# zifeo/distributed-sgd

Measured on NVIDIA H100. Metric: sgd_samples_per_sec, higher is better.
Workload: dtype f64

## Files before the change

distributed_sgd_b200/csrc/dsgd_api.cu:

```cuda
#include "../../include/dsgd.h"

#include <cuda.h>
#include <cuda_runtime.h>
#include <dlfcn.h>
#include <nccl.h>

#include <algorithm>
#include <cmath>
#include <cstdarg>
#include <cstdio>
#include <cstring>
#include <limits>
#include <mutex>
#include <string>
#include <type_traits>
#include <utility>
#include <vector>

#include "dsgd_kernels.cuh"
#include "dsgd_persistent.cuh"
#include "dsgd_stream.cuh"
#include "dsgd_async.cuh"
#include "dsgd_metrics.cuh"
#include "dsgd_calibrate.cuh"
// ... 2599 lines not shown
  if (!nccl().ok) return fail(nullptr, DSGD_ERR_NCCL, "%s", nccl().why.c_str());
  ncclUniqueId u;
  ncclResult_t r = nccl().GetUniqueId(&u);
  if (r != ncclSuccess) return fail(nullptr, DSGD_ERR_NCCL, "ncclGetUniqueId: %s", nccl().GetErrorString(r));
  memcpy(id, &u, sizeof u);
  return DSGD_OK;
}

extern "C" int dsgd_comm_init(dsgd_ctx *ctx, const uint8_t id[DSGD_UNIQUE_ID_BYTES]) {
  if (!ctx) return DSGD_ERR_INVALID;
  NEED(id, DSGD_ERR_INVALID, "dsgd_comm_init: id is NULL");
  NEED(!ctx->comm, DSGD_ERR_STATE, "dsgd_comm_init: communicator already initialised");
  CU(cudaSetDevice(ctx->device));
  ncclUniqueId u;
  memcpy(&u, id, sizeof u);
  NEED(nccl().ok, DSGD_ERR_NCCL, "%s", nccl().why.c_str());
  NC(nccl().CommInitRank(&ctx->comm, ctx->world, u, ctx->rank));
  return DSGD_OK;
}

constexpr int kPCons = 8, kPUpd = 6, kPStages = 8, kPStagePairs = 2560, kPMaxChunks = 128;
using PSmem = PersistSmem<kPCons, kPUpd, kPStages, kPStagePairs, kPMaxChunks>;
constexpr int kPersistForms = 28, kPersistFused = 24;
constexpr bool pf_multi(int f) { return f >= kPersistFused; }
constexpr int pf_weight(int f) { return pf_multi(f) ? kUnweighted : f / 8; }
constexpr bool pf_l1(int f) { return (f & 4) != 0; }
template <int... F>
static void *const *persist_forms(std::integer_sequence<int, F...>) {
  static void *const k[] = {(void *)k_sync_persistent<kPCons, kPUpd, kPStages, kPStagePairs, kPMaxChunks, pf_multi(F),
                                                      (F & 2) != 0, (F & 1) != 0, pf_l1(F), pf_weight(F)>...};
  return k;
}
static void *const *const kPersistKernels = persist_forms(std::make_integer_sequence<int, kPersistForms>{});
static int persist_form(bool multi, bool avg, bool lr_table, bool l1, int weight) {
  if (multi) return kPersistFused + 2 * avg + lr_table;
  return 8 * weight + 4 * l1 + 2 * avg + lr_table;
}
static size_t persist_smem(int f) {
  return sizeof(PSmem) + (pf_weight(f) == kSampleWeighted ? sizeof(PersistSwSmem<kPStages>) : 0);
}
static bool persist_timeline() { static const bool v = getenv("DSGD_PERSIST_TIMELINE") != nullptr; return v; }

static int persist_prepare(dsgd_ctx *ctx, int64_t n_steps) {
  if (!ctx->p_ready) {
    const int64_t nv = (int64_t)ctx->dim + 2;
    const size_t vd = sizeof(double) * (size_t)nv;
    for (int i = 0; i < 2; ++i) CU(ctx->p_wbuf[i].alloc(nv));
    for (int i = 0; i < 3; ++i) {
      CU(ctx->p_gbuf[i].alloc(nv));
      CU(cudaMemsetAsync(ctx->p_gbuf[i], 0, vd, ctx->stream));
      CU(ctx->p_rec[i].alloc(nv));
      CU(cudaMemsetAsync(ctx->p_rec[i], 0, 2 * vd, ctx->stream));
    }
    CU(ctx->p_acc.alloc(3 * kAccStride));
    CU(ctx->p_bar.alloc(4));
    for (int f = 0; f < kPersistForms; ++f)
      CU(cudaFuncSetAttribute(kPersistKernels[f], cudaFuncAttributeMaxDynamicSharedMemorySize, (int)persist_smem(f)));
    ctx->p_ready = true;
  }
  int rc = ctx->p_hinge.grow(ctx, (int64_t)ctx->sm_count * n_steps, 4096 * (int64_t)ctx->sm_count);
  if (rc) return rc;
  if (weighting(ctx) == kSampleWeighted &&
      (rc = ctx->p_hcode.grow(ctx, (int64_t)ctx->sm_count * n_steps, 4096 * (int64_t)ctx->sm_count)))
    return rc;
  return ctx->p_loss_nrm.grow(ctx, 2 * n_steps, 2 * 4096);
}

static int persist_grid(const dsgd_ctx *ctx, int64_t batch) {
  const int g = ctx->grid_limit > 0 ? std::min(ctx->grid_limit, ctx->sm_count) : ctx->sm_count;
  if (cdiv(batch, kMaxRowsPerCta) > g) return 0;
  if (ctx->n_pairs >= (1ll << 31)) return 0;
  return g;
}
static bool persist_multi_fits(const dsgd_ctx *ctx, int G) {
  const int slice = (cdiv(ctx->dim + 1, G) + 31) & ~31;
  return slice <= (kPCons + kPUpd) * 32;
}

static cudaError_t persist_launch(dsgd_ctx *ctx, int form, int G, void **args) {
  void *fn = kPersistKernels[form];
  const size_t smem = persist_smem(form);
  if (ctx->grid_limit > 0) return cudaLaunchKernel(fn, dim3(G), dim3((kPCons + kPUpd + 1) * 32), args, smem, ctx->stream);
  return cudaLaunchCooperativeKernel(fn, dim3(G), dim3((kPCons + kPUpd + 1) * 32), args, smem, ctx->stream);
}

static size_t xblk_stride(const dsgd_ctx *ctx) { return (size_t)(ctx->dim + kReplicaPad); }
static size_t xblk_words(const dsgd_ctx *ctx) { return ((size_t)ctx->dim + 1 + 31) / 32; }
static size_t xblk_bm_offset(const dsgd_ctx *ctx) { return 2 * (size_t)kMaxWorld * 2 * xblk_stride(ctx); }
static size_t xblk_doubles(const dsgd_ctx *ctx) { return xblk_bm_offset(ctx) + (size_t)kMaxWorld * 2 * xblk_words(ctx); }

static int xblk_ensure(dsgd_ctx *ctx) {
  if (ctx->xblk) return DSGD_OK;
  CU(cudaSetDevice(ctx->device));
  CU(ctx->xblk.alloc((int64_t)xblk_doubles(ctx)));
  CU(cudaMemset(ctx->xblk, 0, sizeof(double) * xblk_doubles(ctx)));
  CU(ctx->x_stats.alloc(4));
  CU(cudaMemset(ctx->x_stats, 0, sizeof(unsigned long long) * 4));
  return DSGD_OK;
}

static int xllw_ensure(dsgd_ctx *ctx) {
  if (ctx->x_llw) return DSGD_OK;
  CU(ctx->x_llw.alloc(2 * 2 * (int64_t)xblk_stride(ctx)));
  CU(cudaMemsetAsync(ctx->x_llw, 0, 2 * 2 * sizeof(unsigned long long) * xblk_stride(ctx), ctx->stream));
  return DSGD_OK;
}

static bool xchg_complete(const dsgd_ctx *ctx) {
  if (ctx->world <= 1 || ctx->world > kMaxWorld || !ctx->xblk) return false;
  for (int r = 0; r < ctx->world; ++r)
    if (r != ctx->rank && !ctx->peer_x[r]) return false;
  return true;
}

static int persist_run(dsgd_ctx *ctx, bool multi, const int32_t *samples_dev, int64_t n_per_step, int64_t n_steps,
                       double lr, const double *lrs_host, double *losses_dev) {
  int rc = persist_prepare(ctx, n_steps);
  if (rc) return rc;
  const int G = persist_grid(ctx, n_per_step);
  NEED((uint64_t)G * (uint64_t)(n_steps + 2) < (1ull << 32), DSGD_ERR_INVALID, "dsgd_sync_steps: too many steps for one launch");
  PersistParams pp;
  memset(&pp, 0, sizeof pp);
  pp.rp16 = ctx->rp16; pp.pairs = ctx->pairs; pp.label = ctx->label; pp.samples = samples_dev;
  pp.n_steps = n_steps; pp.batch = (int32_t)n_per_step; pp.dim = ctx->dim;
  pp.wbuf[0] = ctx->p_wbuf[0]; pp.wbuf[1] = ctx->p_wbuf[1];
  for (int i = 0; i < 3; ++i) { pp.gbuf[i] = ctx->p_gbuf[i]; pp.rec[i] = ctx->p_rec[i]; }
  pp.d = ctx->d; pp.acc = ctx->p_acc; pp.bar = ctx->p_bar; pp.hinge = ctx->p_hinge; pp.losses = losses_dev;
  pp.loss_nrm = ctx->p_loss_nrm;
  pp.w_out = ctx->w; pp.w32_out = ctx->w32; pp.scal = ctx->scal;
  pp.abort_flag = reinterpret_cast<int *>(ctx->p_bar + 1);
  CU(cudaMemsetAsync(ctx->p_acc, 0, sizeof(unsigned long long) * 3 * kAccStride, ctx->stream));
  pp.lambda = ctx->lambda; pp.lr = lr; pp.world = 1;
  CU(cudaMemsetAsync(ctx->p_bar, 0, sizeof(unsigned) * 4, ctx->stream));
  if (persist_timeline()) {
    if (!ctx->p_tl) CU(ctx->p_tl.alloc(kTlWords));
    CU(cudaMemsetAsync(ctx->p_tl, 0, sizeof(long long) * kTlWords, ctx->stream));
    pp.tl = ctx->p_tl;
  }
  if (!multi) {
    k_rec_init<<<cdiv(ctx->dim, 256), 256, 0, ctx->stream>>>(ctx->w, ctx->dim, ctx->p_rec[0], ctx->p_rec[1], ctx->p_rec[2]);
    LAUNCHED();
    pp.k_den = 1.0;
    pp.timeout_cycles = 4000000000ll;
  } else {
    CU(cudaMemcpyAsync(ctx->p_wbuf[0], ctx->w, sizeof(double) * (size_t)ctx->dim, cudaMemcpyDeviceToDevice, ctx->stream));
    pp.k_den = (double)ctx->world;
    pp.timeout_cycles = 20000000000ll;
    pp.world = ctx->world; pp.rank = ctx->rank; pp.step_base = ctx->x_step;
    pp.xstride = (int)xblk_stride(ctx);
    pp.xwords = (int)xblk_words(ctx);
    for (int r = 0; r < ctx->world; ++r) {
      unsigned long long *blk = reinterpret_cast<unsigned long long *>((r == ctx->rank) ? ctx->xblk.p : ctx->peer_x[r].p);
      pp.xval[r] = blk;
      pp.xbm[r] = blk + xblk_bm_offset(ctx);
    }
    if ((rc = xllw_ensure(ctx))) return rc;
    pp.llw[0] = ctx->x_llw;
    pp.llw[1] = ctx->x_llw + 2 * xblk_stride(ctx);
    pp.xstats = ctx->x_stats;
  }
  if (ctx->avg_on) pp.avg = ctx->avg;
  if (lrs_host) {
    if ((rc = ctx->lrs.grow(ctx, n_steps, 1024))) return rc;
    CU(cudaMemcpyAsync(ctx->lrs, lrs_host, sizeof(double) * (size_t)n_steps, cudaMemcpyHostToDevice, ctx->stream));
    pp.lrs = ctx->lrs;
    pp.lr = 0.0;
  }
  void *args[] = {&pp};
  const bool l1 = !multi && ctx->lambda1 > 0.0;
  pp.lambda1 = l1 ? ctx->lambda1 : 0.0;
  pp.w_pos = ctx->cw_pos; pp.w_neg = ctx->cw_neg;
  const int weight = multi ? kUnweighted : weighting(ctx);
  if (weight == kSampleWeighted) { pp.sw = ctx->sw; pp.hcode = ctx->p_hcode; }
  const int form = persist_form(multi, ctx->avg_on, lrs_host != nullptr, l1, weight);
  cudaError_t launch_err = cudaSuccess;
  profiled(ctx, [&] { launch_err = persist_launch(ctx, form, G, args); });
  CU(launch_err);
  LAUNCHED();
  if (ctx->avg_on) ctx->avg_n += n_steps;
  if (multi) {
    ctx->x_step += n_steps + 6;
    ctx->x_steps_run += n_steps;
  }
  return DSGD_OK;
// ... 694 lines not shown
```

distributed_sgd_b200/csrc/dsgd_fixed.cuh:

```cuda
#pragma once
#include <cuda_runtime.h>
#include <stdint.h>

namespace dsgd {

constexpr int kAccStride = 16;
constexpr int kAccLimbs = 5;
constexpr int kAccWords = 2 * kAccLimbs + 1;
static_assert(kAccWords + 1 <= kAccStride, "acc_read loads the accumulator and one pad word");
__device__ __forceinline__ void red_add_u64(unsigned long long *p, unsigned long long v) {
  asm volatile("red.relaxed.gpu.global.add.u64 [%0], %1;" ::"l"(p), "l"(v) : "memory");
}
template <class Put>
__device__ __forceinline__ void acc_cut(double a, Put &&put) {
  double F[kAccLimbs - 1];
#pragma unroll
  for (int i = 0; i < kAccLimbs - 1; ++i) F[i] = floor(a * __longlong_as_double((1023ll + 40 * i) << 52));
  put(kAccLimbs - 1, F[0]);
#pragma unroll
  for (int i = 1; i < kAccLimbs - 1; ++i) put(kAccLimbs - 1 - i, F[i] - F[i - 1] * 0x1p40);
  put(0, rint(a * 0x1p160) - F[kAccLimbs - 2] * 0x1p40);
}
__device__ __forceinline__ void acc_push_one(unsigned long long *limbs, unsigned long long *ovf, double v) {
  if (!(fabs(v) < 4503599627370496.0)) {
    red_add_u64(ovf, 1ull);
    return;
  }
  const bool neg = v < 0.0;
  acc_cut(fabs(v), [&](int k, double limb) {
    if (limb != 0.0) {
      const unsigned long long u = (unsigned long long)(long long)limb;
      red_add_u64(limbs + k, neg ? (0ull - u) : u);
    }
  });
}
__device__ __forceinline__ void acc_push(unsigned long long *acc, double sd, double sn) {
  acc_push_one(acc, acc + 2 * kAccLimbs, sd);
  acc_push_one(acc + kAccLimbs, acc + 2 * kAccLimbs, sn);
}
__device__ __forceinline__ double acc_limb(unsigned long long q, int k) {
  return (double)(long long)q * __longlong_as_double((long long)(1023 - 160 + 40 * (k % kAccLimbs)) << 52);
}
__device__ __forceinline__ void acc_load(const unsigned long long *acc, int lane, unsigned long long &q0, unsigned long long &q1) {
  q0 = 0; q1 = 0;
  if (lane < (kAccWords + 1) / 2)
    asm volatile("ld.relaxed.gpu.global.v2.u64 {%0, %1}, [%2];" : "=l"(q0), "=l"(q1) : "l"(acc + 2 * lane) : "memory");
}
__device__ __forceinline__ void acc_sum(unsigned long long q0, unsigned long long q1, int lane, double &sd, double &sn) {
  const double lo = acc_limb(q0, 2 * lane), hi = acc_limb(q1, 2 * lane + 1), pair = lo + hi;
  const double s01 = __shfl_sync(0xffffffffu, pair, 0), s23 = __shfl_sync(0xffffffffu, pair, 1);
  const double s4 = __shfl_sync(0xffffffffu, lo, 2), n0 = __shfl_sync(0xffffffffu, hi, 2);
  const double n12 = __shfl_sync(0xffffffffu, pair, 3), n34 = __shfl_sync(0xffffffffu, pair, 4);
  sd = (s01 + s23) + s4;
  sn = (n0 + n12) + n34;
  if (__any_sync(0xffffffffu, lane == kAccWords / 2 && q0 != 0)) {
    sd = __longlong_as_double(0x7ff8000000000000ll);
    sn = sd;
  }
}
__device__ __forceinline__ void acc_read(const unsigned long long *acc, int lane, double &sd, double &sn) {
  unsigned long long q0, q1;
  acc_load(acc, lane, q0, q1);
  acc_sum(q0, q1, lane, sd, sn);
}
__device__ __forceinline__ void acc_load_l1(const unsigned long long *acc, int lane, unsigned long long &q, unsigned long long &o) {
  q = 0; o = 0;
  if (lane < kAccLimbs) asm volatile("ld.relaxed.gpu.global.u64 %0, [%1];" : "=l"(q) : "l"(acc + kAccWords + lane) : "memory");
  if (lane == 0) asm volatile("ld.relaxed.gpu.global.u64 %0, [%1];" : "=l"(o) : "l"(acc + 2 * kAccLimbs) : "memory");
}
__device__ __forceinline__ double acc_sum_l1(unsigned long long q, unsigned long long o, int lane) {
  const double v = acc_limb(q, lane);
  const double v0 = __shfl_sync(0xffffffffu, v, 0), v1 = __shfl_sync(0xffffffffu, v, 1), v2 = __shfl_sync(0xffffffffu, v, 2);
  const double v3 = __shfl_sync(0xffffffffu, v, 3), v4 = __shfl_sync(0xffffffffu, v, 4);
  const double a = (((v4 + v3) + v2) + v1) + v0;
  return __shfl_sync(0xffffffffu, o, 0) != 0ull ? __longlong_as_double(0x7ff8000000000000ll) : a;
}
__device__ __forceinline__ double acc_read_l1(const unsigned long long *acc, int lane) {
  unsigned long long q, o;
  acc_load_l1(acc, lane, q, o);
  return acc_sum_l1(q, o, lane);
}

constexpr int kLossLimbs = kAccLimbs + 1;
constexpr int kLossAccWords = kLossLimbs + 1;
constexpr unsigned long long kLimbMask = (1ull << 40) - 1;
__device__ __forceinline__ void acc_carry(unsigned long long (&q)[kLossLimbs]) {
#pragma unroll
  for (int i = 0; i < kLossLimbs - 1; ++i) {
    q[i + 1] += q[i] >> 40;
    q[i] &= kLimbMask;
  }
}
__device__ __forceinline__ void acc_add_local(unsigned long long (&lim)[kLossLimbs], unsigned long long &ovf, double v) {
  if (!(v >= 0.0 && v < 4503599627370496.0)) { ++ovf; return; }
  acc_cut(v, [&](int k, double limb) { lim[k] += (unsigned long long)(long long)limb; });
  acc_carry(lim);
}
__device__ __forceinline__ void acc_flush_local(unsigned long long *acc, const unsigned long long (&lim)[kLossLimbs],
                                                unsigned long long ovf) {
#pragma unroll
  for (int i = 0; i < kLossLimbs; ++i)
    if (lim[i]) red_add_u64(acc + i, lim[i]);
  if (ovf) red_add_u64(acc + kLossLimbs, ovf);
}
__device__ __forceinline__ double acc_value(const unsigned long long *acc) {
  if (acc[kLossLimbs] != 0ull) return __longlong_as_double(0x7ff8000000000000ll);
  unsigned long long q[kLossLimbs];
#pragma unroll
  for (int i = 0; i < kLossLimbs; ++i) q[i] = acc[i];
  acc_carry(q);
  double s = (double)q[kLossLimbs - 1] * 0x1p40;
#pragma unroll
  for (int i = kLossLimbs - 2; i >= 0; --i) s += (double)q[i] * __longlong_as_double((long long)(1023 - 160 + 40 * i) << 52);
  return s;
}

}
```

distributed_sgd_b200/csrc/dsgd_persistent.cuh:

```cuda
#pragma once
#include <cuda_runtime.h>
#include <stdint.h>

#include <type_traits>

#include "dsgd_fixed.cuh"
#include "dsgd_kernels.cuh"

namespace dsgd {

constexpr int kMaxWorld = 8;

struct PersistParams {
  const uint32_t *rp16;
  const uint2 *pairs;
  const int8_t *label;
  const int32_t *samples;
  int64_t n_steps;
  int32_t batch;
  int32_t dim;
  double *wbuf[2];
  double *gbuf[3];
  double2 *rec[3];
  const double *d;
// ... 77 lines not shown
__device__ __forceinline__ void st_relaxed_gpu(unsigned *p, unsigned v) {
  asm volatile("st.relaxed.gpu.global.u32 [%0], %1;" ::"l"(p), "r"(v) : "memory");
}
__device__ __forceinline__ void fence_acq_rel_gpu() { asm volatile("fence.acq_rel.gpu;" ::: "memory"); }
__device__ __forceinline__ void named_bar_sync(int id, int n_threads) {
  asm volatile("bar.sync %0, %1;" ::"r"(id), "r"(n_threads) : "memory");
}
__device__ __forceinline__ void named_bar_arrive(int id, int n_threads) {
  asm volatile("bar.arrive %0, %1;" ::"r"(id), "r"(n_threads) : "memory");
}
__device__ __forceinline__ long long global_ns() {
  long long t;
  asm volatile("mov.u64 %0, %%globaltimer;" : "=l"(t));
  return t;
}

__device__ __forceinline__ void ll_store(unsigned long long *dst, double v, unsigned tag) {
  const unsigned long long bits = (unsigned long long)__double_as_longlong(v);
  const unsigned long long w0 = (bits & 0xffffffffull) | ((unsigned long long)tag << 32);
  const unsigned long long w1 = (bits >> 32) | ((unsigned long long)tag << 32);
  asm volatile("st.relaxed.sys.global.v2.u64 [%0], {%1, %2};" ::"l"(dst), "l"(w0), "l"(w1) : "memory");
}
__device__ __forceinline__ bool ll_try_load(const unsigned long long *src, unsigned tag, double &v) {
  unsigned long long w0, w1;
  asm volatile("ld.relaxed.sys.global.v2.u64 {%0, %1}, [%2];" : "=l"(w0), "=l"(w1) : "l"(src) : "memory");
  if ((unsigned)(w0 >> 32) != tag || (unsigned)(w1 >> 32) != tag) return false;
  v = __longlong_as_double((long long)((w0 & 0xffffffffull) | (w1 << 32)));
  return true;
}
__device__ __forceinline__ void ll_store32(unsigned long long *dst, unsigned v, unsigned tag) {
  const unsigned long long w = (unsigned long long)v | ((unsigned long long)tag << 32);
  asm volatile("st.relaxed.sys.global.u64 [%0], %1;" ::"l"(dst), "l"(w) : "memory");
}
__device__ __forceinline__ bool ll_try_load32(const unsigned long long *src, unsigned tag, unsigned &v) {
  unsigned long long w;
  asm volatile("ld.relaxed.sys.global.u64 %0, [%1];" : "=l"(w) : "l"(src) : "memory");
  v = (unsigned)w;
  return (unsigned)(w >> 32) == tag;
}

__device__ __forceinline__ double apply_update(double wv, double graw, double c, bool add_c, double k_den, double lr) {
  double v = filt(graw);
  if (v != 0.0) {
    if (add_c) v = filt(v + c);
    if (v != 0.0) {
      const double mean = (k_den == 1.0) ? v : filt(v / k_den);
      const double step = filt(mean * lr);
      wv = filt(wv - step);
    }
  }
  return wv;
}

__device__ __forceinline__ bool grid_barrier_arrive_wait(unsigned *bar, unsigned target, int *abort_flag, long long timeout) {
  red_release_gpu_add(bar, 1u);
  const long long t0 = clock64();
  unsigned spins = 0;
  bool ok = true;
  while ((int)(ld_relaxed_gpu(bar) - target) < 0) {
    if ((++spins & 1023u) == 0u && (clock64() - t0 > timeout || *(volatile int *)abort_flag)) {
      *(volatile int *)abort_flag = 1;
      ok = false;
      break;
    }
  }
  return ok;
}

constexpr int kChunkPairs = 128;
static_assert(kChunkPairs == kFoldPairs, "a listed row's chunks are the chunks of the row fold");
constexpr uint32_t kChunkGlobal = 1u << 31;
constexpr int kMaxRowsPerCta = 32;
constexpr int kRowBarFirst = 5, kRowBars = 11;

template <int kMaxChunks>
struct StageMeta {
  int n_rows;
  int n_chunks;
  int n_multi;
  int two_pass;
  int n_pairs;
  int row_y[kMaxRowsPerCta];
  uint32_t row_b[kMaxRowsPerCta];
  int row_len[kMaxRowsPerCta];
  short row_first[kMaxRowsPerCta];
  short row_nch[kMaxRowsPerCta];
  signed char row_bar[kMaxRowsPerCta];
  uint32_t ch_off[kMaxChunks];
  short ch_n[kMaxChunks];
  short ch_row[kMaxChunks];
  double part[kMaxChunks];
};

template <int kStages>
struct PersistSwSmem {
  double row_c[kStages][kMaxRowsPerCta];
  unsigned long long code;
};

template <int kCons, int kUpd, int kStages, int kStagePairs, int kMaxChunks>
struct PersistSmem {
  uint2 ring[kStages][kStagePairs];
  StageMeta<kMaxChunks> meta[kStages];
  uint64_t full[kStages];
  uint64_t empty[kStages];
  uint64_t c_bar[2];
  uint64_t u_bar;
  double red[kCons + kUpd][2];
  double c_val[2];
  double nrm_val[2];
  unsigned hinge_acc;
  int ok;
  long long tl_warp[kCons + kUpd];
};

#define DSGD_TL(slot_)                                                                        \
  do {                                                                                        \
    if (p.tl && blockIdx.x == 0 && lane == 0 && t < 256) p.tl[t * 16 + (slot_)] = clock64(); \
  } while (0)
constexpr int kTlSteps = 4, kTlFirst = 100, kTlCtas = 160, kTlPerCta = 4;
constexpr int kTlWords = 256 * 16 + kTlSteps * kTlCtas * kTlPerCta;

template <bool kL1 = false>
struct FetchLocal {
  const double2 *R;
  uint64_t *cbar;
  unsigned cpar;
  const double *cval;
  int *abort_flag;
  long long timeout;
  double k_den, lr;
  double tau = 0.0;
  double c = 0.0;
  bool add_c = false, have_c = false, good = true;
  __device__ __forceinline__ void need_c() {
    if (!have_c) {
      mbar_wait(cbar, cpar, abort_flag, timeout);
      c = *(volatile const double *)cval;
      add_c = (c != 0.0) && (fabs(c) > kEps);
      have_c = true;
    }
  }
  __device__ __forceinline__ void get4(const uint2 (&pr)[4], double (&wv)[4]) {
    double2 r[4];
#pragma unroll
    for (int u = 0; u < 4; ++u) {
      r[u] = make_double2(0.0, 0.0);
      if (pr[u].y << 1) r[u] = __ldcg(&R[pr[u].x]);
    }
    need_c();
#pragma unroll
    for (int u = 0; u < 4; ++u) {
      wv[u] = apply_update(r[u].x, r[u].y, c, add_c, k_den, lr);
      if constexpr (kL1) wv[u] = soft_threshold(wv[u], tau);
    }
  }
  __device__ __forceinline__ double get1(uint32_t col) {
    need_c();
    const double2 r = __ldcg(&R[col]);
    const double wv = apply_update(r.x, r.y, c, add_c, k_den, lr);
    if constexpr (kL1) return soft_threshold(wv, tau);
    return wv;
  }
// ... 301 lines not shown

  double lr = p.lr;
  const int64_t base = kMulti ? p.step_base : 0;
  unsigned phase = 0;
  const int n_upd = G * kUpd * 32;
  const int u0 = blockIdx.x * kUpd * 32 + ((int)threadIdx.x - kCons * 32);
  const int K = p.world, me = p.rank;
  const int slice = ((p.dim + 1 + G - 1) / G + 31) & ~31;
  const int j_col = blockIdx.x * slice + (int)threadIdx.x;
  const bool col_act = kMulti && (int)threadIdx.x < slice && j_col <= p.dim;
  const int col_word = j_col >> 5;
  unsigned long long st_val = 0, st_bm = 0;
  constexpr int kUpdCols = 2;
  double wreg[kUpdCols], dreg[kUpdCols];
  double areg[kUpdCols];
  int ttl[kUpdCols];
  bool gnz[kUpdCols];
#pragma unroll
  for (int i = 0; i < kUpdCols; ++i) {
    wreg[i] = dreg[i] = 0.0;
    areg[i] = 0.0;
    ttl[i] = 0;
    gnz[i] = false;
    if constexpr (!kMulti) {
      const int j = u0 + i * n_upd;
      if (is_upd && j < p.dim) {
        wreg[i] = __ldcg(&p.rec[2][j].x);
        dreg[i] = __ldg(&p.d[j]);
        if constexpr (kAvg) areg[i] = p.avg[j];
      }
    }
  }
  if constexpr (kMulti) {
    if (col_act && j_col < p.dim) {
      wreg[0] = __ldcg(&p.wbuf[0][j_col]);
      dreg[0] = __ldg(&p.d[j_col]);
      if constexpr (kAvg) areg[0] = p.avg[j_col];
    }
  }

  uint2 pre[4];
  auto prefetch = [&](int64_t tn) {
    const int st = (int)tn & (kStages - 1);
    const auto &mt = sm.meta[st];
    mbar_wait(&sm.full[st], (unsigned)(((unsigned)tn / kStages) & 1u), p.abort_flag, p.timeout_cycles);
#pragma unroll
    for (int u = 0; u < 4; ++u) pre[u] = make_uint2(0u, 0u);
    if (warp < mt.n_chunks) chunk_pairs(mt, &sm.ring[st][0], p.pairs, warp, lane, pre);
  };
  if (!kMulti && is_cons && S > 0) prefetch(0);

  int gi_prev = (int)((base + 2) % 3), gi_cur = (int)(base % 3), gi_next = (int)((base + 1) % 3);
  int ti_prev = 2, ti_cur = 0, ti_next = 1;
  for (int64_t T = base; T <= base + S; ++T) {
    const int64_t t = T - base;
    const bool first = (t == 0), last = (t == S);
    const double *Gprev = p.gbuf[gi_prev];
    double *Gcur = p.gbuf[gi_cur];
    double *Gzero = p.gbuf[gi_next];
    const unsigned long long *acc_prev = p.acc + (size_t)ti_prev * kAccStride;
    unsigned long long *acc_cur = p.acc + (size_t)ti_cur * kAccStride;
    unsigned long long *acc_next = p.acc + (size_t)ti_next * kAccStride;
    const double2 *Rprev = p.rec[ti_prev];
    double2 *Rcur = p.rec[ti_cur];
    double2 *Rnext = p.rec[ti_next];
    const unsigned c_par = (unsigned)((t >> 1) & 1);
    const bool tl_cta = p.tl && t >= kTlFirst && t < kTlFirst + kTlSteps && blockIdx.x < kTlCtas;
    long long *tl_rec = tl_cta ? p.tl + 256 * 16 + ((t - kTlFirst) * kTlCtas + blockIdx.x) * kTlPerCta : nullptr;
    long long *tl_row = (p.tl && blockIdx.x == 0 && t < 256) ? p.tl + t * 16 : nullptr;
    bool ok = true;
    double lr_next = lr;
    if constexpr (kLrTable) {
      if (!last) lr_next = __ldg(&p.lrs[t]);
    }
    if (warp == 0) DSGD_TL(0);

    double gv[kUpdCols];
#pragma unroll
    for (int i = 0; i < kUpdCols; ++i) {
      const int j = u0 + i * n_upd;
      gv[i] = (!kMulti && is_upd && j < p.dim) ? __ldcg(&Rprev[j].y) : 0.0;
    }

    if (warp == kCons && !first) {
      double c_prev, nrm_prev, l1_prev = 0.0;
      if (kMulti && t == 1) {
        c_prev = p.scal[kScalC];
        nrm_prev = p.scal[kScalNrm2];
      } else {
        unsigned long long q0, q1, ql = 0, ol = 0;
        acc_load(acc_prev, lane, q0, q1);
        if constexpr (kL1) acc_load_l1(acc_prev, lane, ql, ol);
        double sd, sn;
        acc_sum(q0, q1, lane, sd, sn);
        c_prev = p.lambda * 2.0 * sd;
        nrm_prev = sn;
        if constexpr (kL1) l1_prev = acc_sum_l1(ql, ol, lane);
      }
      if (blockIdx.x == 0 && lane < (kL1 ? kAccStride : kAccWords)) acc_next[lane] = 0ull;
      if (lane == 0) {
        sm.c_val[t & 1] = c_prev;
        sm.nrm_val[t & 1] = nrm_prev;
        mbar_arrive(&sm.c_bar[t & 1]);
        if (!kMulti && p.losses && blockIdx.x == 0) {
          p.loss_nrm[t - 1] = nrm_prev;
          if constexpr (kL1) p.loss_nrm[S + t - 1] = l1_prev;
        }
      }
      __syncwarp();
      DSGD_TL(9);
    }
    double pd = 0.0, pn = 0.0;
    double pa = 0.0;
    const double tau = (kL1 && !first) ? lr * p.lambda1 : 0.0;
    auto publish_partial = [&]() {
      pd = warp_sum(pd);
      pn = warp_sum(pn);
      if constexpr (kL1) pa = warp_sum(pa);
      if (lane == 0) {
        sm.red[warp][0] = pd;
        sm.red[warp][1] = pn;
        if constexpr (kL1) sm.red[warp - kCons][0] = pa;
        mbar_arrive(&sm.u_bar);
      }
      if (warp == kCons) {
        mbar_wait(&sm.u_bar, (unsigned)(t & 1), p.abort_flag, p.timeout_cycles);
        if (lane == 0) {
          double sd = 0.0, sn = 0.0;
#pragma unroll
          for (int i = kMulti ? 0 : kCons; i < kCons + kUpd; ++i) { sd += sm.red[i][0]; sn += sm.red[i][1]; }
          if (sd != 0.0 || sn != 0.0) acc_push(acc_cur, sd, sn);
          if constexpr (kL1) {
            double sa = 0.0;
#pragma unroll
            for (int i = 0; i < kUpd; ++i) sa += sm.red[i][0];
            if (sa != 0.0) acc_push_one(acc_cur + kAccWords, acc_cur + 2 * kAccLimbs, sa);
          }
        }
        __syncwarp();
      }
    };

    if constexpr (kMulti) {
      unsigned long long *LWcur = p.llw[T & 1];
      const int parp = (int)((T + 1) & 1);
      const unsigned gtag = (unsigned)T;
      const unsigned wtag = (unsigned)(T + 1);
      if ((int)threadIdx.x < slice) {
        if (first) {
          if (col_act) {
            if (j_col < p.dim) ll_store(LWcur + 2 * (size_t)j_col, wreg[0], wtag);
            Gzero[j_col] = 0.0;
          }
        } else {
          double own = 0.0;
          if (col_act) {
            own = __ldcg(&Gprev[j_col]);
            if (j_col < p.dim) own = filt(own);
          }
          const unsigned my_bits = __ballot_sync(0xffffffffu, own != 0.0);
          const bool warp_act = blockIdx.x * slice + (warp << 5) <= p.dim;
          if (warp_act) {
            const size_t vslot = 2 * (((size_t)me * 2 + parp) * p.xstride + (size_t)j_col);
            const size_t bslot = ((size_t)me * 2 + parp) * p.xwords + (size_t)col_word;
            for (int k = 0; k < K; ++k) {
              if (k == me) continue;
              if (lane == 0) ll_store32(p.xbm[k] + bslot, my_bits, gtag);
              if (own != 0.0) ll_store(p.xval[k] + vslot, own, gtag);
            }
            if (lane == 0) { st_bm += 1; st_val += (unsigned)__popc(my_bits); }
          }
          if (warp == 0) DSGD_TL(11);
          if (warp_act) {
            double raw[kMaxWorld];
            unsigned need = 0;
            double wn = wreg[0];
            const unsigned long long *bm0 = p.xbm[me] + (size_t)parp * p.xwords + (size_t)col_word;
            const unsigned long long *vl0 = p.xval[me] + 2 * ((size_t)parp * p.xstride + (size_t)j_col);
            unsigned bits[kMaxWorld];
            unsigned pend = 0;
#pragma unroll
            for (int k = 0; k < kMaxWorld; ++k) {
              raw[k] = (k == me) ? own : 0.0;
              bits[k] = 0u;
              if (k < K && k != me) pend |= 1u << k;
            }
            {
              unsigned spins = 0;
              const long long t0 = clock64();
// ... 129 lines not shown
        }
      } else {
        mbar_wait(&sm.c_bar[t & 1], c_par, p.abort_flag, p.timeout_cycles);
        const double c_prev = *(volatile double *)&sm.c_val[t & 1];
        const bool add_c = (c_prev != 0.0) && (fabs(c_prev) > kEps);
#pragma unroll
        for (int i = 0; i < kUpdCols; ++i) {
          const int j = u0 + i * n_upd;
          if (j < p.dim) {
            if (gv[i] != 0.0) {
              wreg[i] = apply_update(wreg[i], gv[i], c_prev, add_c, p.k_den, lr);
              ttl[i] = 3;
            }
            if constexpr (kL1) {
              const double wt = soft_threshold(wreg[i], tau);
              if (__double_as_longlong(wt) != __double_as_longlong(wreg[i])) { wreg[i] = wt; ttl[i] = 3; }
              pa += fabs(wreg[i]);
            }
            if (ttl[i] > 0) { Rcur[j].x = wreg[i]; --ttl[i]; }
            if (gnz[i]) Rnext[j].y = 0.0;
            gnz[i] = gv[i] != 0.0;
            if constexpr (kAvg) if (!first) areg[i] = areg[i] + wreg[i];
            pd += filt(wreg[i] * dreg[i]);
            pn += wreg[i] * wreg[i];
          }
        }
        for (int j = u0 + kUpdCols * n_upd; j < p.dim; j += n_upd) {
          const double2 r = __ldcg(&Rprev[j]);
          double wn = apply_update(r.x, r.y, c_prev, add_c, p.k_den, lr);
          if constexpr (kL1) {
            wn = soft_threshold(wn, tau);
            pa += fabs(wn);
          }
          Rcur[j].x = wn;
          Rnext[j].y = 0.0;
          if constexpr (kAvg) if (!first) p.avg[j] = p.avg[j] + wn;
          pd += filt(wn * __ldg(&p.d[j]));
          pn += wn * wn;
        }
        if (warp == kCons) DSGD_TL(10);
        publish_partial();
      }
    }

    if (!ok) *(volatile int *)&sm.ok = 0;
    if (tl_row && lane == 0) sm.tl_warp[warp] = clock64();
    if (!kMulti && is_cons) {
      named_bar_arrive(3, kSyncThreads);
      if (t + 1 < S) prefetch(t + 1);
    } else {
      named_bar_sync(3, kSyncThreads);
    }
    ++phase;
    if (threadIdx.x == kCons * 32) {
      if (tl_row) {
        long long mc = 0, mu = 0;
        for (int i = 0; i < kCons; ++i) mc = max(mc, sm.tl_warp[i]);
        for (int i = kCons; i < kCons + kUpd; ++i) mu = max(mu, sm.tl_warp[i]);
        tl_row[13] = mc;
        tl_row[14] = mu;
      }
      unsigned h = 0;
      if (!last) {
        h = sm.hinge_acc;
        if constexpr (kMulti) {
          if (h) red_add_f64(&Gcur[p.dim], (double)h);
          if (blockIdx.x == 0) red_add_f64(&Gcur[p.dim], (double)B * 4294967296.0);
        }
        sm.hinge_acc = 0u;
      }
      if (tl_rec) tl_rec[0] = global_ns();
      else if (tl_row) tl_row[6] = clock64();
      bool bar_ok = grid_barrier_arrive_wait(p.bar, phase * (unsigned)G, p.abort_flag, p.timeout_cycles);
      if (*(volatile int *)&sm.ok == 0) { *(volatile int *)p.abort_flag = 1; bar_ok = false; }
      sm.ok = bar_ok ? 1 : 0;
      if (tl_rec) tl_rec[1] = global_ns();
      else if (tl_row) tl_row[7] = clock64();
      if (!kMulti && !last && p.losses) p.hinge[(size_t)t * G + blockIdx.x] = h;
      if constexpr (kWeight == kSampleWeighted) {
        if (!last) {
          if (p.losses) p.hcode[(size_t)t * G + blockIdx.x] = swm.code;
          swm.code = 0ull;
        }
      }
    }
    named_bar_sync(4, kSyncThreads);
    if (*(volatile int *)&sm.ok == 0) return;
    if constexpr (kLrTable) lr = lr_next;
    { const int a = gi_prev; gi_prev = gi_cur; gi_cur = gi_next; gi_next = a; }
    { const int a = ti_prev; ti_prev = ti_cur; ti_cur = ti_next; ti_next = a; }
  }

  if (blockIdx.x == 0 && warp == kCons && S > 0) {
    double sd, sn;
    acc_read(p.acc + (size_t)ti_prev * kAccStride, lane, sd, sn);
    double l1 = 0.0;
    if constexpr (kL1) l1 = acc_read_l1(p.acc + (size_t)ti_prev * kAccStride, lane);
    if (lane == 0) {
      p.scal[kScalC] = p.lambda * 2.0 * sd;
      p.scal[kScalNrm2] = sn;
      if constexpr (kL1) p.scal[kScalL1] = l1;
    }
  }
  if constexpr (!kMulti && kWeight != kSampleWeighted) {
    if (p.losses) {
      for (int64_t s = (int64_t)blockIdx.x * (kCons + kUpd) + warp; s < S; s += (int64_t)G * (kCons + kUpd)) {
        unsigned h = 0;
        if constexpr (kWeight == kClassWeighted) {
          unsigned hn = 0;
          for (int b = lane; b < G; b += 32) {
            const unsigned v = __ldcg(&p.hinge[s * G + b]);
            h += v & 0xffffu;
            hn += v >> 16;
          }
          h = __reduce_add_sync(0xffffffffu, h);
          hn = __reduce_add_sync(0xffffffffu, hn);
          if (lane == 0) {
            const double hp_w = p.w_pos * (double)h, hn_w = p.w_neg * (double)hn;
            double pen = p.lambda * __ldcg(&p.loss_nrm[s]);
            if constexpr (kL1) pen = pen + p.lambda1 * __ldcg(&p.loss_nrm[S + s]);
            p.losses[s] = pen + (hp_w + hn_w) / (double)B;
          }
        } else {
          for (int b = lane; b < G; b += 32) h += __ldcg(&p.hinge[s * G + b]);
          h = __reduce_add_sync(0xffffffffu, h);
          if (lane == 0) {
            if constexpr (kL1)
              p.losses[s] = p.lambda * __ldcg(&p.loss_nrm[s]) + p.lambda1 * __ldcg(&p.loss_nrm[S + s]) + (double)h / (double)B;
            else
              p.losses[s] = p.lambda * __ldcg(&p.loss_nrm[s]) + (double)h / (double)B;
          }
        }
      }
    }
  }
  if constexpr (kMulti) {
    const unsigned long long *LW = p.llw[(base + S) & 1];
    const unsigned wtag = (unsigned)(base + S + 1);
    const int n_all = G * kSyncThreads;
    for (int j = blockIdx.x * kSyncThreads + threadIdx.x; j < p.dim; j += n_all) {
      double wv = 0.0;
      ll_try_load(LW + 2 * (size_t)j, wtag, wv);
      p.w_out[j] = wv;
      p.w32_out[j] = (float)wv;
    }
    if (p.xstats && lane == 0 && (st_val | st_bm)) {
      atomicAdd(&p.xstats[0], st_val);
      atomicAdd(&p.xstats[1], st_bm);
    }
    if constexpr (kAvg) {
      if (col_act && j_col < p.dim) p.avg[j_col] = areg[0];
    }
  } else if (is_upd) {
    const double2 *Rfin = p.rec[ti_prev];
#pragma unroll
    for (int i = 0; i < kUpdCols; ++i) {
      const int j = u0 + i * n_upd;
      if (j < p.dim) {
        p.w_out[j] = wreg[i];
        p.w32_out[j] = (float)wreg[i];
        if constexpr (kAvg) p.avg[j] = areg[i];
      }
    }
    for (int j = u0 + kUpdCols * n_upd; j < p.dim; j += n_upd) {
      const double wv = __ldcg(&Rfin[j]).x;
      p.w_out[j] = wv;
      p.w32_out[j] = (float)wv;
    }
  }
  if constexpr (kWeight == kSampleWeighted) {
    if (p.losses) {
      for (int64_t s = (int64_t)blockIdx.x * (kCons + kUpd) + warp; s < S; s += (int64_t)G * (kCons + kUpd)) {
        unsigned long long lim[kLossLimbs] = {0, 0, 0, 0, 0, 0}, ovf = 0;
        for (int i = lane; i < B; i += 32) {
          const int b = i % G, m = i / G;
          const unsigned code = (unsigned)(__ldcg(&p.hcode[s * G + b]) >> (2 * m)) & 3u;
          const int32_t id = __ldg(&p.samples[s * B + i]);
          const double c = (__ldg(&p.label[id]) > 0 ? p.w_pos : p.w_neg) * __ldg(&p.sw[id]);
          acc_add_local(lim, ovf, c * (double)code);
        }
#pragma unroll
        for (int o = 16; o > 0; o >>= 1) {
#pragma unroll
          for (int k = 0; k < kLossLimbs; ++k) lim[k] += __shfl_xor_sync(0xffffffffu, lim[k], o);
          ovf += __shfl_xor_sync(0xffffffffu, ovf, o);
        }
        if (lane == 0) {
          unsigned long long q[kLossAccWords];
#pragma unroll
          for (int k = 0; k < kLossLimbs; ++k) q[k] = lim[k];
          q[kLossLimbs] = ovf;
          double pen = p.lambda * __ldcg(&p.loss_nrm[s]);
          if constexpr (kL1) pen = pen + p.lambda1 * __ldcg(&p.loss_nrm[S + s]);
          p.losses[s] = pen + acc_value(q) / (double)B;
        }
      }
    }
  }
}

__global__ void __launch_bounds__(256) k_rec_init(const double *__restrict__ w, int dim, double2 *__restrict__ rec0,
                                                  double2 *__restrict__ rec1, double2 *__restrict__ rec2) {
  const int j = blockIdx.x * blockDim.x + threadIdx.x;
  if (j < dim) {
    const double2 r = make_double2(w[j], 0.0);
    rec0[j] = r;
    rec1[j] = r;
    rec2[j] = r;
  }
}

}
```

Before: 76.54 million.

## Split persistent accumulator into scale and norm lines, overlap norm work with barrier

In the single-device persistent kernel, the fixed-point accumulator is split. The scale term keeps its own 3-way rotated line, and the squared-norm and L1 sums move to a separate 4-way rotated set of lines. Norm pushes and block 0's read, write and clear of older norm lines now run while the grid barrier is being waited on, and the scale limbs are prefetched right after the barrier so the consumer warp does no global load before signalling. The aim is to take norm accumulation and loss bookkeeping off the critical path between steps, at the cost of more rotation state, extra accumulator lines, and more delicate ordering for the last two steps' losses.

```diff
diff --git a/distributed_sgd_b200/csrc/dsgd_api.cu b/distributed_sgd_b200/csrc/dsgd_api.cu
--- a/distributed_sgd_b200/csrc/dsgd_api.cu
+++ b/distributed_sgd_b200/csrc/dsgd_api.cu
@@ -2675,7 +2675,7 @@
       CU(ctx->p_rec[i].alloc(nv));
       CU(cudaMemsetAsync(ctx->p_rec[i], 0, 2 * vd, ctx->stream));
     }
-    CU(ctx->p_acc.alloc(3 * kAccStride));
+    CU(ctx->p_acc.alloc(kAccLines * kAccStride));
     CU(ctx->p_bar.alloc(4));
     for (int f = 0; f < kPersistForms; ++f)
       CU(cudaFuncSetAttribute(kPersistKernels[f], cudaFuncAttributeMaxDynamicSharedMemorySize, (int)persist_smem(f)));
@@ -2752,7 +2752,7 @@
   pp.loss_nrm = ctx->p_loss_nrm;
   pp.w_out = ctx->w; pp.w32_out = ctx->w32; pp.scal = ctx->scal;
   pp.abort_flag = reinterpret_cast<int *>(ctx->p_bar + 1);
-  CU(cudaMemsetAsync(ctx->p_acc, 0, sizeof(unsigned long long) * 3 * kAccStride, ctx->stream));
+  CU(cudaMemsetAsync(ctx->p_acc, 0, sizeof(unsigned long long) * kAccLines * kAccStride, ctx->stream));
   pp.lambda = ctx->lambda; pp.lr = lr; pp.world = 1;
   CU(cudaMemsetAsync(ctx->p_bar, 0, sizeof(unsigned) * 4, ctx->stream));
   if (persist_timeline()) {
diff --git a/distributed_sgd_b200/csrc/dsgd_fixed.cuh b/distributed_sgd_b200/csrc/dsgd_fixed.cuh
--- a/distributed_sgd_b200/csrc/dsgd_fixed.cuh
+++ b/distributed_sgd_b200/csrc/dsgd_fixed.cuh
@@ -8,9 +8,14 @@
 constexpr int kAccLimbs = 5;
 constexpr int kAccWords = 2 * kAccLimbs + 1;
 static_assert(kAccWords + 1 <= kAccStride, "acc_read loads the accumulator and one pad word");
+constexpr int kAccRot = 3;
+constexpr int kNrmRot = 4;
+constexpr int kAccLines = kAccRot + kNrmRot;
+constexpr int kCWords = kAccLimbs + 1;
 __device__ __forceinline__ void red_add_u64(unsigned long long *p, unsigned long long v) {
   asm volatile("red.relaxed.gpu.global.add.u64 [%0], %1;" ::"l"(p), "l"(v) : "memory");
 }
+__device__ __forceinline__ bool acc_fits(double v) { return fabs(v) < 4503599627370496.0; }
 template <class Put>
 __device__ __forceinline__ void acc_cut(double a, Put &&put) {
   double F[kAccLimbs - 1];
@@ -22,7 +27,7 @@
   put(0, rint(a * 0x1p160) - F[kAccLimbs - 2] * 0x1p40);
 }
 __device__ __forceinline__ void acc_push_one(unsigned long long *limbs, unsigned long long *ovf, double v) {
-  if (!(fabs(v) < 4503599627370496.0)) {
+  if (!acc_fits(v)) {
     red_add_u64(ovf, 1ull);
     return;
   }
@@ -81,6 +86,44 @@
   return acc_sum_l1(q, o, lane);
 }
 
+__device__ __forceinline__ unsigned long long *acc_line(unsigned long long *acc, int i) { return acc + i * kAccStride; }
+__device__ __forceinline__ unsigned long long *nrm_line(unsigned long long *acc, int i) { return acc + (kAccRot + i) * kAccStride; }
+__device__ __forceinline__ void acc_push_c(unsigned long long *line, double sd) {
+  if (sd != 0.0) acc_push_one(line, line + kAccLimbs, sd);
+}
+__device__ __forceinline__ void acc_push_nrm(unsigned long long *line, double sn, double sa) {
+  if (sn != 0.0) acc_push_one(line + kAccLimbs, line + 2 * kAccLimbs, sn);
+  if (sa != 0.0) acc_push_one(line + kAccWords, line + 2 * kAccLimbs, sa);
+}
+__device__ __forceinline__ void acc_load_c(const unsigned long long *line, unsigned long long (&q)[kCWords]) {
+#pragma unroll
+  for (int i = 0; i < kCWords / 2; ++i)
+    asm volatile("ld.relaxed.gpu.global.v2.u64 {%0, %1}, [%2];" : "=l"(q[2 * i]), "=l"(q[2 * i + 1]) : "l"(line + 2 * i) : "memory");
+}
+__device__ __forceinline__ double acc_sum_c(const unsigned long long (&q)[kCWords]) {
+  if (q[kAccLimbs] != 0ull) return __longlong_as_double(0x7ff8000000000000ll);
+  return ((acc_limb(q[0], 0) + acc_limb(q[1], 1)) + (acc_limb(q[2], 2) + acc_limb(q[3], 3))) + acc_limb(q[4], 4);
+}
+__device__ __forceinline__ void acc_zero_c(unsigned long long *line, int lane) {
+  if (lane < kCWords) line[lane] = 0ull;
+}
+__device__ __forceinline__ void acc_read_nrm(const unsigned long long *line, double &sn, double &sa) {
+  unsigned long long q[kAccStride - kAccLimbs + 1];
+#pragma unroll
+  for (int i = 0; i < (kAccStride - kAccLimbs + 1) / 2; ++i)
+    asm volatile("ld.relaxed.gpu.global.v2.u64 {%0, %1}, [%2];" : "=l"(q[2 * i]), "=l"(q[2 * i + 1])
+                 : "l"(line + kAccLimbs - 1 + 2 * i) : "memory");
+  const unsigned long long *n = q + 1, *a = q + 1 + kAccWords - kAccLimbs;
+  sn = (acc_limb(n[0], 0) + (acc_limb(n[1], 1) + acc_limb(n[2], 2))) + (acc_limb(n[3], 3) + acc_limb(n[4], 4));
+  sa = (((acc_limb(a[4], 4) + acc_limb(a[3], 3)) + acc_limb(a[2], 2)) + acc_limb(a[1], 1)) + acc_limb(a[0], 0);
+  if (q[1 + kAccLimbs] != 0ull) sn = sa = __longlong_as_double(0x7ff8000000000000ll);
+}
+__device__ __forceinline__ void acc_zero_nrm(unsigned long long *line) {
+#pragma unroll
+  for (int i = 0; i < (kAccStride - kAccLimbs + 1) / 2; ++i)
+    asm volatile("st.relaxed.gpu.global.v2.u64 [%0], {%1, %1};" ::"l"(line + kAccLimbs - 1 + 2 * i), "l"(0ull) : "memory");
+}
+
 constexpr int kLossLimbs = kAccLimbs + 1;
 constexpr int kLossAccWords = kLossLimbs + 1;
 constexpr unsigned long long kLimbMask = (1ull << 40) - 1;
diff --git a/distributed_sgd_b200/csrc/dsgd_persistent.cuh b/distributed_sgd_b200/csrc/dsgd_persistent.cuh
--- a/distributed_sgd_b200/csrc/dsgd_persistent.cuh
+++ b/distributed_sgd_b200/csrc/dsgd_persistent.cuh
@@ -153,19 +153,27 @@
   return wv;
 }
 
-__device__ __forceinline__ bool grid_barrier_arrive_wait(unsigned *bar, unsigned target, int *abort_flag, long long timeout) {
+template <class Wait>
+__device__ __forceinline__ bool grid_barrier_arrive_wait(unsigned *bar, unsigned target, int *abort_flag, long long timeout,
+                                                         Wait &&while_waiting) {
   red_release_gpu_add(bar, 1u);
+  unsigned v = ld_relaxed_gpu(bar);
+  while_waiting();
   const long long t0 = clock64();
   unsigned spins = 0;
   bool ok = true;
-  while ((int)(ld_relaxed_gpu(bar) - target) < 0) {
+  while ((int)(v - target) < 0) {
     if ((++spins & 1023u) == 0u && (clock64() - t0 > timeout || *(volatile int *)abort_flag)) {
       *(volatile int *)abort_flag = 1;
       ok = false;
       break;
     }
+    v = ld_relaxed_gpu(bar);
   }
   return ok;
+}
+__device__ __forceinline__ bool grid_barrier_arrive_wait(unsigned *bar, unsigned target, int *abort_flag, long long timeout) {
+  return grid_barrier_arrive_wait(bar, target, abort_flag, timeout, [] {});
 }
 
 constexpr int kChunkPairs = 128;
@@ -210,6 +218,7 @@
   double red[kCons + kUpd][2];
   double c_val[2];
   double nrm_val[2];
+  double nrm_part[2];
   unsigned hinge_acc;
   int ok;
   long long tl_warp[kCons + kUpd];
@@ -617,15 +626,16 @@
 
   int gi_prev = (int)((base + 2) % 3), gi_cur = (int)(base % 3), gi_next = (int)((base + 1) % 3);
   int ti_prev = 2, ti_cur = 0, ti_next = 1;
+  unsigned long long cq[kCWords];
   for (int64_t T = base; T <= base + S; ++T) {
     const int64_t t = T - base;
     const bool first = (t == 0), last = (t == S);
     const double *Gprev = p.gbuf[gi_prev];
     double *Gcur = p.gbuf[gi_cur];
     double *Gzero = p.gbuf[gi_next];
-    const unsigned long long *acc_prev = p.acc + (size_t)ti_prev * kAccStride;
-    unsigned long long *acc_cur = p.acc + (size_t)ti_cur * kAccStride;
-    unsigned long long *acc_next = p.acc + (size_t)ti_next * kAccStride;
+    const unsigned long long *acc_prev = acc_line(p.acc, ti_prev);
+    unsigned long long *acc_cur = acc_line(p.acc, ti_cur);
+    unsigned long long *acc_next = acc_line(p.acc, ti_next);
     const double2 *Rprev = p.rec[ti_prev];
     double2 *Rcur = p.rec[ti_cur];
     double2 *Rnext = p.rec[ti_next];
@@ -648,29 +658,27 @@
     }
 
     if (warp == kCons && !first) {
-      double c_prev, nrm_prev, l1_prev = 0.0;
-      if (kMulti && t == 1) {
-        c_prev = p.scal[kScalC];
-        nrm_prev = p.scal[kScalNrm2];
+      double c_prev, nrm_prev = 0.0;
+      if constexpr (kMulti) {
+        if (t == 1) {
+          c_prev = p.scal[kScalC];
+          nrm_prev = p.scal[kScalNrm2];
+        } else {
+          double sd, sn;
+          acc_read(acc_prev, lane, sd, sn);
+          c_prev = p.lambda * 2.0 * sd;
+          nrm_prev = sn;
+        }
+        if (blockIdx.x == 0 && lane < kAccWords) acc_next[lane] = 0ull;
       } else {
-        unsigned long long q0, q1, ql = 0, ol = 0;
-        acc_load(acc_prev, lane, q0, q1);
-        if constexpr (kL1) acc_load_l1(acc_prev, lane, ql, ol);
-        double sd, sn;
-        acc_sum(q0, q1, lane, sd, sn);
-        c_prev = p.lambda * 2.0 * sd;
-        nrm_prev = sn;
-        if constexpr (kL1) l1_prev = acc_sum_l1(ql, ol, lane);
-      }
-      if (blockIdx.x == 0 && lane < (kL1 ? kAccStride : kAccWords)) acc_next[lane] = 0ull;
+        c_prev = p.lambda * 2.0 * acc_sum_c(cq);
+        if (tl_row && lane == 0) tl_row[8] = clock64();
+        if (blockIdx.x == 0) acc_zero_c(acc_next, lane);
+      }
       if (lane == 0) {
         sm.c_val[t & 1] = c_prev;
-        sm.nrm_val[t & 1] = nrm_prev;
+        if constexpr (kMulti) sm.nrm_val[t & 1] = nrm_prev;
         mbar_arrive(&sm.c_bar[t & 1]);
-        if (!kMulti && p.losses && blockIdx.x == 0) {
-          p.loss_nrm[t - 1] = nrm_prev;
-          if constexpr (kL1) p.loss_nrm[S + t - 1] = l1_prev;
-        }
       }
       __syncwarp();
       DSGD_TL(9);
@@ -694,12 +702,22 @@
           double sd = 0.0, sn = 0.0;
 #pragma unroll
           for (int i = kMulti ? 0 : kCons; i < kCons + kUpd; ++i) { sd += sm.red[i][0]; sn += sm.red[i][1]; }
-          if (sd != 0.0 || sn != 0.0) acc_push(acc_cur, sd, sn);
-          if constexpr (kL1) {
+          if constexpr (kMulti) {
+            if (sd != 0.0 || sn != 0.0) acc_push(acc_cur, sd, sn);
+          } else {
             double sa = 0.0;
-#pragma unroll
-            for (int i = 0; i < kUpd; ++i) sa += sm.red[i][0];
-            if (sa != 0.0) acc_push_one(acc_cur + kAccWords, acc_cur + 2 * kAccLimbs, sa);
+            if constexpr (kL1) {
+#pragma unroll
+              for (int i = 0; i < kUpd; ++i) sa += sm.red[i][0];
+            }
+            if (!acc_fits(sd) || !acc_fits(sn) || !acc_fits(sa)) sd = sn = __longlong_as_double(0x7ff8000000000000ll);
+            acc_push_c(acc_cur, sd);
+            if (last) {
+              acc_push_nrm(nrm_line(p.acc, (int)(t & (kNrmRot - 1))), sn, sa);
+            } else {
+              sm.nrm_part[0] = sn;
+              sm.nrm_part[1] = sa;
+            }
           }
         }
         __syncwarp();
@@ -935,6 +953,8 @@
       named_bar_sync(3, kSyncThreads);
     }
     ++phase;
+#pragma unroll
+    for (int i = 0; i < kCWords; ++i) cq[i] = 0ull;
     if (threadIdx.x == kCons * 32) {
       if (tl_row) {
         long long mc = 0, mu = 0;
@@ -954,7 +974,23 @@
       }
       if (tl_rec) tl_rec[0] = global_ns();
       else if (tl_row) tl_row[6] = clock64();
-      bool bar_ok = grid_barrier_arrive_wait(p.bar, phase * (unsigned)G, p.abort_flag, p.timeout_cycles);
+      auto while_waiting = [&]() {
+        if constexpr (!kMulti) {
+          if (p.losses && !last) {
+            acc_push_nrm(nrm_line(p.acc, (int)(t & (kNrmRot - 1))), sm.nrm_part[0], sm.nrm_part[1]);
+            if (blockIdx.x == 0 && t >= 2) {
+              unsigned long long *nl = nrm_line(p.acc, (int)((t - 2) & (kNrmRot - 1)));
+              double n2, n1;
+              acc_read_nrm(nl, n2, n1);
+              p.loss_nrm[t - 2] = n2;
+              if constexpr (kL1) p.loss_nrm[S + t - 2] = n1;
+              acc_zero_nrm(nl);
+            }
+          }
+        }
+      };
+      bool bar_ok = grid_barrier_arrive_wait(p.bar, phase * (unsigned)G, p.abort_flag, p.timeout_cycles, while_waiting);
+      if (!kMulti && !last) acc_load_c(acc_cur, cq);
       if (*(volatile int *)&sm.ok == 0) { *(volatile int *)p.abort_flag = 1; bar_ok = false; }
       sm.ok = bar_ok ? 1 : 0;
       if (tl_rec) tl_rec[1] = global_ns();
@@ -976,19 +1012,36 @@
 
   if (blockIdx.x == 0 && warp == kCons && S > 0) {
     double sd, sn;
-    acc_read(p.acc + (size_t)ti_prev * kAccStride, lane, sd, sn);
     double l1 = 0.0;
-    if constexpr (kL1) l1 = acc_read_l1(p.acc + (size_t)ti_prev * kAccStride, lane);
+    if constexpr (kMulti) {
+      acc_read(acc_line(p.acc, ti_prev), lane, sd, sn);
+    } else {
+      unsigned long long q[kCWords];
+      acc_load_c(acc_line(p.acc, ti_prev), q);
+      sd = acc_sum_c(q);
+      acc_read_nrm(nrm_line(p.acc, (int)(S & (kNrmRot - 1))), sn, l1);
+    }
     if (lane == 0) {
       p.scal[kScalC] = p.lambda * 2.0 * sd;
       p.scal[kScalNrm2] = sn;
       if constexpr (kL1) p.scal[kScalL1] = l1;
     }
   }
+  auto loss_norms = [&](int64_t s, double &n2, double &n1) {
+    n1 = 0.0;
+    if (s >= S - 2) {
+      acc_read_nrm(nrm_line(p.acc, (int)(s & (kNrmRot - 1))), n2, n1);
+    } else {
+      n2 = __ldcg(&p.loss_nrm[s]);
+      if constexpr (kL1) n1 = __ldcg(&p.loss_nrm[S + s]);
+    }
+  };
   if constexpr (!kMulti && kWeight != kSampleWeighted) {
     if (p.losses) {
       for (int64_t s = (int64_t)blockIdx.x * (kCons + kUpd) + warp; s < S; s += (int64_t)G * (kCons + kUpd)) {
         unsigned h = 0;
+        double n2, n1;
+        loss_norms(s, n2, n1);
         if constexpr (kWeight == kClassWeighted) {
           unsigned hn = 0;
           for (int b = lane; b < G; b += 32) {
@@ -1000,8 +1053,8 @@
           hn = __reduce_add_sync(0xffffffffu, hn);
           if (lane == 0) {
             const double hp_w = p.w_pos * (double)h, hn_w = p.w_neg * (double)hn;
-            double pen = p.lambda * __ldcg(&p.loss_nrm[s]);
-            if constexpr (kL1) pen = pen + p.lambda1 * __ldcg(&p.loss_nrm[S + s]);
+            double pen = p.lambda * n2;
+            if constexpr (kL1) pen = pen + p.lambda1 * n1;
             p.losses[s] = pen + (hp_w + hn_w) / (double)B;
           }
         } else {
@@ -1009,9 +1062,9 @@
           h = __reduce_add_sync(0xffffffffu, h);
           if (lane == 0) {
             if constexpr (kL1)
-              p.losses[s] = p.lambda * __ldcg(&p.loss_nrm[s]) + p.lambda1 * __ldcg(&p.loss_nrm[S + s]) + (double)h / (double)B;
+              p.losses[s] = p.lambda * n2 + p.lambda1 * n1 + (double)h / (double)B;
             else
-              p.losses[s] = p.lambda * __ldcg(&p.loss_nrm[s]) + (double)h / (double)B;
+              p.losses[s] = p.lambda * n2 + (double)h / (double)B;
           }
         }
       }
@@ -1054,6 +1107,8 @@
   if constexpr (kWeight == kSampleWeighted) {
     if (p.losses) {
       for (int64_t s = (int64_t)blockIdx.x * (kCons + kUpd) + warp; s < S; s += (int64_t)G * (kCons + kUpd)) {
+        double n2, n1;
+        loss_norms(s, n2, n1);
         unsigned long long lim[kLossLimbs] = {0, 0, 0, 0, 0, 0}, ovf = 0;
         for (int i = lane; i < B; i += 32) {
           const int b = i % G, m = i / G;
@@ -1073,8 +1128,8 @@
 #pragma unroll
           for (int k = 0; k < kLossLimbs; ++k) q[k] = lim[k];
           q[kLossLimbs] = ovf;
-          double pen = p.lambda * __ldcg(&p.loss_nrm[s]);
-          if constexpr (kL1) pen = pen + p.lambda1 * __ldcg(&p.loss_nrm[S + s]);
+          double pen = p.lambda * n2;
+          if constexpr (kL1) pen = pen + p.lambda1 * n1;
           p.losses[s] = pen + acc_value(q) / (double)B;
         }
       }
```

Result: no change. 76.35 million, median of 6 (-0.3%).
